# VincentStimper/normalizing-flows

Measured on NVIDIA H100. Metric: samples/sec forward_kld, 32-layer RQ-NSF d=64 batch=65536, higher is better.
Workload: dtype f32

## Files before the change

### normalizing-flows_b200/csrc/nfb_fused_rqs.cu

```cuda
#include <type_traits>

#include "nfb_kernels.h"
#include "nfb_spline.cuh"

namespace nfb {

constexpr int kRows = kFusedTileRows;
constexpr int kCons = 256;
constexpr int kFusedThreads = kCons + 128;
constexpr int kProducerRegs = 24, kConsumerRegs = 240;
constexpr uint32_t kTileA = 8192;
constexpr uint32_t kSlotBytes = 32768;
constexpr uint32_t kSlots = 3;
constexpr uint32_t kOffW = 8 * kTileA;
constexpr uint32_t kOffX = kOffW + kSlots * kSlotBytes;
constexpr int kStgLd = 52;
constexpr uint32_t kStgBytes = kRows * kStgLd * 4;
constexpr uint32_t kOffStg = kOffX + kRows * 64 * 4;
constexpr uint32_t kOffMisc = kOffStg + 2 * kStgBytes;
constexpr uint32_t kOffBars = kOffMisc + 4 * kRows * 4;
constexpr uint32_t kNumBars = 10;
constexpr uint32_t kOffUnitQ = kOffBars + kNumBars * 8;
constexpr uint32_t kFusedSmem = kOffUnitQ + 32;
static_assert(kFusedSmem <= 232448, "shared memory budget");
static_assert(2 * kFusedFeaturesPerChunk * 24 * 64 * 4 <= (int)kSlotBytes, "final-layer record must fit a ring slot");

constexpr int kBarWFull = 0 , kBarWEmpty = 3 , kBarUnit = 6 ;

__device__ __forceinline__ uint32_t xs_index(int r, int c) { return r * 64 + (c ^ (r & 31)); }

__device__ __forceinline__ uint32_t a_chunk_off(int r, int c8) {
    return (r >> 3) * 1024 + (r & 7) * 128 + ((c8 ^ (r & 7)) << 4);
}

__device__ __forceinline__ void st_shared_v4(uint32_t addr, uint32_t a, uint32_t b, uint32_t c,
                                             uint32_t d) {
    asm volatile("st.shared.v4.b32 [%0], {%1,%2,%3,%4};" ::"r"(addr), "r"(a), "r"(b), "r"(c), "r"(d)
                 : "memory");
}
__device__ __forceinline__ void st_shared_b32(uint32_t addr, uint32_t v) {
    asm volatile("st.shared.b32 [%0], %1;" ::"r"(addr), "r"(v) : "memory");
}
__device__ __forceinline__ void cons_bar_sync() {
    asm volatile("bar.sync 1, %0;" ::"n"(kCons) : "memory");
}
constexpr int kBarStgFull = 2, kBarStgFree = 3;
template <int ID> __device__ __forceinline__ void stg_bar_arrive() {
    __threadfence_block();
    asm volatile("bar.arrive %0, %1;" ::"n"(ID), "n"(kCons) : "memory");
}
template <int ID> __device__ __forceinline__ void stg_bar_wait() {
    asm volatile("bar.sync %0, %1;" ::"n"(ID), "n"(kCons) : "memory");
}
__device__ __forceinline__ void mbar_arrive_if(uint32_t bar, bool pred) {
    asm volatile("{\n\t.reg .pred p;\n\tsetp.ne.b32 p, %1, 0;\n\t@p mbarrier.arrive.shared::cta.b64 _, [%0];\n\t}"
                 ::"r"(bar), "r"((uint32_t)pred) : "memory");
}

__device__ __forceinline__ void split_store8(const float* v, uint32_t t0, uint32_t t1, uint32_t off) {
    uint32_t h[4], l[4];
#pragma unroll
    for (int i = 0; i < 4; ++i) {
        const float a = v[2 * i], b = v[2 * i + 1];
        h[i] = pack_f16x2(a, b);
        const float2 hf = unpack_f16x2(h[i]);
        l[i] = pack_f16x2(a - hf.x, b - hf.y);
    }
    st_shared_v4(t0 + off, h[0], h[1], h[2], h[3]);
    st_shared_v4(t1 + off, l[0], l[1], l[2], l[3]);
}
template <typename T> __device__ __forceinline__ T uniform(T v) {
    return (T)__shfl_sync(0xffffffffu, (int)v, 0);
}
__device__ __forceinline__ float pow2i(int e) { return __uint_as_float((uint32_t)(127 + e) << 23); }

struct MmaOps { uint32_t a_hi, a_lo, w_hi, w_lo; bool first; uint32_t on, slabs; };
template <int SLABS, bool QUAD, int NREG, bool FIRST = false>
__device__ __forceinline__ void mma_record(float (&acc)[NREG], const MmaOps& x) {
    static_assert(NREG == 32 || NREG == 48, "N = 64 or 96");
    static_assert(!FIRST || NREG == 48, "an opening record of its own: the final layer's N = 96 products");
    const uint64_t ah = wgmma_desc(x.a_hi), al = wgmma_desc(x.a_lo), bh = wgmma_desc(x.w_hi), bl = wgmma_desc(x.w_lo);
    auto pass = [&](uint64_t a, uint64_t b, bool opens) {
#pragma unroll
        for (int s = 0; s < SLABS; ++s) {
            const uint32_t sd = opens && s == 0 && x.first ? 0u : 1u;
            if constexpr (NREG == 32) wgmma_f16_n64(acc, a + 2 * s, b + 2 * s, sd);
            else if (FIRST && opens && s == 0) wgmma_f16_n96_zero(acc, a, b);
            else wgmma_f16_n96(acc, a + 2 * s, b + 2 * s, FIRST ? 1u : sd);
        }
    };
    pass(ah, bh, true);
    pass(al, bh, false);
    pass(ah, bl, false);
    if constexpr (QUAD) pass(al, bl, false);
}

enum { kClkClaim,
       kClkLoad,
       kClkLu,
       kClkHidRing,
       kClkHidMma,
       kClkHidEpi,
       kClkFinRing,
       kClkFinMma,
       kClkFinTail,
       kClkFinStage,
       kClkFinSpline,
       kClkStore,
       kClkProdEmpty,
       kClkProdOther,
       kClkUnits,
       kClkCount };
template <int P> using ClkPhase = std::integral_constant<int, P>;
#ifdef NFB_PHASE_CLOCKS
__device__ unsigned long long g_phase_clocks[3][kClkCount];
struct PhaseClock {
    uint32_t last, sum[kClkCount];
    __device__ PhaseClock() {
        last = (uint32_t)clock64();
#pragma unroll
        for (int i = 0; i < kClkCount; ++i) sum[i] = 0;
    }
    template <int P> __device__ __forceinline__ void stamp() {
        const uint32_t t = (uint32_t)clock64();
        sum[P] += t - last;
        last = t;
    }
    __device__ void flush(int role) const {
#pragma unroll
        for (int i = 0; i < kClkCount; ++i) atomicAdd(&g_phase_clocks[role][i], (unsigned long long)sum[i]);
    }
};
#define NFB_CLK_BEGIN() PhaseClock clk
#define NFB_CLK(P) clk.template stamp<P>()
#define NFB_CLK_UNIT() (++clk.sum[kClkUnits])
#define NFB_CLK_END(role, pred) do { if (pred) clk.flush(role); } while (0)
#else
#define NFB_CLK_BEGIN() ((void)0)
#define NFB_CLK(P) ((void)0)
#define NFB_CLK_UNIT() ((void)0)
#define NFB_CLK_END(role, pred) ((void)0)
#endif

template <bool SAMPLE>
__global__ void __launch_bounds__(kFusedThreads, 1) fused_rqs_kernel(const FusedParams p) {
    extern __shared__ __align__(1024) uint8_t smem[];
    const uint32_t sbase = smem_u32(smem);
    const int warp = uniform((int)(threadIdx.x >> 5)), lane = threadIdx.x & 31;
    float* xs = reinterpret_cast<float*>(smem + kOffX);
    float* ldsum = reinterpret_cast<float*>(smem + kOffMisc);
    int* rowexp = reinterpret_cast<int*>(smem + kOffMisc + 3 * kRows * 4);
    float* rowmax = reinterpret_cast<float*>(smem + kOffStg);
    const uint32_t bars = sbase + kOffBars;
    auto bar = [bars](int i) { return bars + 8u * i; };

    if ((sbase & 1023u) != 0) {
        if (threadIdx.x == 0 && p.err) atomicExch(p.err, 900);
        return;
    }
    if (threadIdx.x == 0) {
        for (int i = 0; i < (int)kSlots; ++i) {
            mbar_init(bar(kBarWFull + i), 1);
            mbar_init(bar(kBarWEmpty + i), 2);
        }
        for (int i = 0; i < 4; ++i) mbar_init(bar(kBarUnit + i), 1);
        fence_mbar_init();
    }
    __syncthreads();

    volatile int* unit_q = reinterpret_cast<volatile int*>(smem + kOffUnitQ);
    if (warp >= kCons / 32) {
        setmaxnreg_dec<kProducerRegs>();
        if (warp != kCons / 32) return;
        const long long n_tiles = (p.rows + kRows - 1) / kRows;
        const long long n_units = n_tiles * p.n_layers;
        auto decode = [&](long long u, int& cursor, int& layer, long long& tile) {
            if (!p.wave_order) {
                layer = (int)(u / n_tiles);
                tile = u - (long long)layer * n_tiles;
                return;
            }
            while (cursor + 1 < p.wave_elems && u >= (long long)__ldg(p.wave_order + 2 * (cursor + 1) + 1)) ++cursor;
            const uint32_t w = __ldg(p.wave_order + 2 * cursor);
            layer = (int)(w & 0xffu);
            tile = (long long)(w >> 8) * p.wave_tpg + (u - (long long)__ldg(p.wave_order + 2 * cursor + 1));
        };
        uint32_t slot = 0, par = 0;
        int wcur = 0;
        NFB_CLK_BEGIN();
        for (uint32_t ui = 0;; ++ui) {
            long long u;
            if (p.ticket) {
                int t = 0;
                if (lane == 0) t = atomicAdd(p.ticket, 1);
                u = (long long)__shfl_sync(0xffffffffu, t, 0);
            } else {
                u = (long long)blockIdx.x + (long long)ui * gridDim.x;
            }
            const bool more = u < n_units;
            int ulayer = -1;
            long long utile = 0;
            if (more) decode(u, wcur, ulayer, utile);
            if (lane == 0) {
                unit_q[2 * (ui & 3u)] = ulayer;
                unit_q[2 * (ui & 3u) + 1] = (int)utile;
                mbar_arrive(bar(kBarUnit + (ui & 3u)));
            }
            __syncwarp();
            if (!more) break;
            NFB_CLK_UNIT();
            const FusedLayer& L = p.layers[ulayer];
            const FusedStep* steps = L.steps;
            const int n_steps = L.n_steps;
            const int lu_steps = L.has_lu ? 1 : 0;
            const int reps = (SAMPLE && L.ar_passes > 0) ? L.ar_passes : 1;
            const int total = n_steps ? lu_steps + reps * (n_steps - lu_steps) : 0;
            const uint32_t lu_bytes = L.has_lu ? 2u * 8192u : 0u;
            int s = 0;
            uint32_t off = 0;
            uint32_t bytes = total ? (uint32_t)__ldg(&steps[0].bytes16) << 4 : 0u;
            for (int i = 0; i < total; ++i) {
                int sn = s + 1;
                uint32_t offn = off + bytes;
                if (sn == n_steps) { sn = lu_steps; offn = lu_bytes; }
                const uint32_t nbytes = i + 1 < total ? (uint32_t)__ldg(&steps[sn].bytes16) << 4 : 0u;
                NFB_CLK(kClkProdOther);
                mbar_wait(bar(kBarWEmpty + slot), par ^ 1, p.err, 100 + slot);
                NFB_CLK(kClkProdEmpty);
                if (elect_one_sync()) {
                    mbar_expect_tx(bar(kBarWFull + slot), bytes);
                    bulk_g2s(sbase + kOffW + slot * kSlotBytes, L.wstream + off, bytes, bar(kBarWFull + slot));
                }
                __syncwarp();
                s = sn;
                off = offn;
                bytes = nbytes;
                if (++slot == kSlots) { slot = 0; par ^= 1; }
            }
        }
        NFB_CLK(kClkProdOther);
        NFB_CLK_END(2, lane == 0);
        return;
    }

    setmaxnreg_inc<kConsumerRegs>();
    const int et = threadIdx.x;
    const int wg = uniform(et >> 7);
    const int wl = warp & 3;
    const int ra = 16 * wl + (lane >> 2);
    const int rb = ra + 8;
    const int cq = 2 * (lane & 3);
    const uint32_t aA = sbase;
    float* stg0 = reinterpret_cast<float*>(smem + kOffStg);
    uint32_t slot = 0, wpar = 0;
    NFB_CLK_BEGIN();

    for (uint32_t ui = 0;; ++ui) {
        mbar_wait(bar(kBarUnit + (ui & 3u)), (ui >> 2) & 1u, p.err, 600 + (int)(ui & 3u));
        const int layer = uniform(unit_q[2 * (ui & 3u)]);
        const long long tile = uniform(unit_q[2 * (ui & 3u) + 1]);
        if (layer < 0) break;
        NFB_CLK_UNIT();
        const FusedLayer& L = p.layers[layer];
        const int D = L.D;
        auto own = [&](int q) { return uniform((int)L.own[wg][q]); };
        const int n_steps = uniform(L.n_steps), lu_steps = uniform(L.has_lu ? 1 : 0);
        const int n_hidden = uniform(L.n_hidden), n_pairs = uniform(L.n_chunks >> 1);
        int sidx = 0;
        auto hand_back = [&](auto arrivals, int s, bool pred) {
#pragma unroll
            for (int i = 0; i < decltype(arrivals)::value; ++i) mbar_arrive_if(bar(kBarWEmpty + s), pred && (et & 127) == 0);
        };
        auto walk_records = [&](auto issue, auto arrivals, auto clk_ring, auto clk_mma, int& prev, auto open,
                                auto retire) {
            auto record = [&](auto first) {
                union { uint2 raw; FusedStep s; } st;
                st.raw = __ldg(reinterpret_cast<const uint2*>(L.steps) + sidx);
                st.raw.x = uniform(st.raw.x);
                st.raw.y = uniform(st.raw.y);
                sidx = sidx + 1 == n_steps ? lu_steps : sidx + 1;
                NFB_CLK(decltype(clk_mma)::value);
                mbar_wait(bar(kBarWFull + slot), wpar, p.err, 220 + slot);
                NFB_CLK(decltype(clk_ring)::value);
                wgmma_fence();
                const bool last = issue(st.s, first);
                if constexpr (decltype(first)::value) NFB_CLK(decltype(clk_mma)::value);
                wgmma_wait<1>();
                hand_back(arrivals, prev < 0 ? 0 : prev, prev >= 0);
                if constexpr (decltype(first)::value) NFB_CLK(kClkFinTail);
                prev = (int)slot;
                if (++slot == kSlots) { slot = 0; wpar ^= 1; }
                return last;
            };
            bool last = false;
            if constexpr (decltype(open)::value) {
                last = record(std::true_type());
                retire();
            }
            while (!last) last = record(std::false_type());
        };
        auto run_records = [&](auto issue, auto arrivals, auto clk_ring, auto clk_mma) {
            int prev = -1;
            walk_records(issue, arrivals, clk_ring, clk_mma, prev, std::false_type(), [] {});
            wgmma_wait<0>();
            hand_back(arrivals, prev, true);
            NFB_CLK(decltype(clk_mma)::value);
        };
        auto half_ops = [&](const FusedStep& s, int h, bool live) {
            const uint32_t kc = h ? s.kc1 : s.kc, fl = h ? s.flags1 : s.flags;
            const uint32_t w = sbase + kOffW + slot * kSlotBytes + ((fl & kStepHalf) ? 0u : (uint32_t)h * s.n8 * 1024u);
            return MmaOps{aA + kc * kTileA, aA + (4 + kc) * kTileA, w, w + ((uint32_t)s.bytes16 << 3), (fl & kStepFirst) != 0,
                          (uint32_t)(live && !(fl & kStepSkip)), 4u - ((fl >> kStepSlabShift) & 3u)};
        };
        auto run_slice = [&](auto& acc, bool live, auto quad, auto clk_ring, auto clk_mma) {
            run_records([&](const FusedStep& s, auto) {
                const MmaOps x = half_ops(s, wg, live);
                if (x.on) mma_record<4, decltype(quad)::value>(acc, x);
                wgmma_commit();
                return ((wg ? s.flags1 : s.flags) & kStepLast) != 0;
            }, std::integral_constant<int, 1>(), clk_ring, clk_mma);
            wgmma_hold(acc);
        };
        using NoQuad = std::integral_constant<bool, false>;

        float* zdst = p.zout + (long long)layer * p.z_stride;
        const float* zsrc = layer == 0 ? p.zin : p.zout + (long long)(layer - 1) * p.z_stride;
        const long long row0 = tile * kRows;
        const int r = et & (kRows - 1);
        const int rq = et >> 6;
        const long long grow = row0 + r;
        const bool row_live = grow < p.rows;

        if (layer > 0) {
            if (lane == 0) {
                const int* flag = p.progress + tile;
                int seen;
                const long long t0 = clock64();
                do {
                    asm volatile("ld.acquire.gpu.global.s32 %0, [%1];" : "=r"(seen) : "l"(flag) : "memory");
                    if (seen < layer && clock64() - t0 > 4000000000LL) fail_timeout(p.err, 500);
                } while (seen < layer);
            }
            __syncwarp();
            {
                int seen;
                asm volatile("ld.acquire.gpu.global.s32 %0, [%1];" : "=r"(seen) : "l"(p.progress + tile) : "memory");
                if (seen < layer) fail_timeout(p.err, 501);
            }
        }
        if (layer == 0 && p.in_ready) {
            const int need = (int)min(row0 + kRows, p.rows);
            if (lane == 0) {
                int seen;
                const long long t0 = clock64();
                do {
                    asm volatile("ld.acquire.sys.global.s32 %0, [%1];" : "=r"(seen) : "l"(p.in_ready) : "memory");
                    if (seen < need && clock64() - t0 > 20000000000LL) fail_timeout(p.err, 510);
                } while (seen < need);
            }
            __syncwarp();
            {
                int seen;
                asm volatile("ld.acquire.sys.global.s32 %0, [%1];" : "=r"(seen) : "l"(p.in_ready) : "memory");
                if (seen < need) fail_timeout(p.err, 511);
            }
        }
        NFB_CLK(kClkClaim);
        float lq_old = 0.f;
        if (rq == 2 && row_live && (layer > 0 || p.accumulate)) lq_old = __ldcg(p.logq + grow);
        if (D == 64) {
            float4 v[kRows * 16 / kCons];
#pragma unroll
            for (int k = 0; k < kRows * 16 / kCons; ++k) {
                const int i4 = et + k * kCons, rr = i4 >> 4;
                const long long gr = row0 + rr;
                v[k] = gr < p.rows ? __ldcg(reinterpret_cast<const float4*>(zsrc + gr * 64) + (i4 & 15))
                                   : make_float4(0.f, 0.f, 0.f, 0.f);
            }
#pragma unroll
            for (int k = 0; k < kRows * 16 / kCons; ++k) {
                const int i4 = et + k * kCons, rr = i4 >> 4, c0 = (i4 & 15) * 4;
                xs[xs_index(rr, c0)] = v[k].x;
                xs[xs_index(rr, c0 + 1)] = v[k].y;
                xs[xs_index(rr, c0 + 2)] = v[k].z;
                xs[xs_index(rr, c0 + 3)] = v[k].w;
                float m = fmaxf(fmaxf(fabsf(v[k].x), fabsf(v[k].y)), fmaxf(fabsf(v[k].z), fabsf(v[k].w)));
                m = fmaxf(m, __shfl_xor_sync(0xffffffffu, m, 1));
                m = fmaxf(m, __shfl_xor_sync(0xffffffffu, m, 2));
                m = fmaxf(m, __shfl_xor_sync(0xffffffffu, m, 4));
                m = fmaxf(m, __shfl_xor_sync(0xffffffffu, m, 8));
                if ((et & 15) == 0) rowmax[rr] = m;
            }
        } else {
            for (int i = et; i < kRows * D; i += kCons) {
                const int rr = i / D, cc = i - rr * D;
                const long long gr = row0 + rr;
                xs[xs_index(rr, cc)] = gr < p.rows ? __ldcg(zsrc + gr * D + cc) : 0.f;
            }
        }
        cons_bar_sync();
        auto set_row_exp = [&](float zmax) {
            int e = (int)((__float_as_uint(zmax) >> 23) & 0xffu) - 126;
            rowexp[r] = max(0, min(126, e));
        };
        if (rq == 0) {
            float zmax = 0.f;
            if (D == 64) zmax = rowmax[r];
            else
                for (int c = 0; c < D; ++c) zmax = fmaxf(zmax, fabsf(xs[xs_index(r, c)]));
            set_row_exp(zmax);
        }
        cons_bar_sync();
        auto ru = [&](float s, int row) { return s * pow2i(-rowexp[row]); };
        auto ruinv = [&](float s, int row) { return s * pow2i(rowexp[row]); };
        auto get_x = [&](int c) -> float { return xs[xs_index(r, c)]; };
        auto put_y = [&](int c, float y) { xs[xs_index(r, c)] = y; };
        const int ar = et >> 2, aq = et & 3;
        auto store_a = [&](auto value, float sc_base) {
            const float sc = ru(sc_base, ar);
            float v[16];
#pragma unroll
            for (int j = 0; j < 16; ++j) v[j] = value(aq * 16 + j) * sc;
#pragma unroll
            for (int g = 0; g < 2; ++g) split_store8(v + 8 * g, aA, aA + 4 * kTileA, a_chunk_off(ar, 2 * aq + g));
            fence_proxy_async_smem();
            cons_bar_sync();
        };
        auto build_a_net = [&]() {
            store_a([&](int k) {
                const int c = L.in_idx[k];
                return c >= 0 ? xs[xs_index(ar, c)] : 0.f;
            }, L.a_sc[1]);
        };
        float ladsum = 0.f, lad_even = 0.f;
        const bool folded = uniform(!SAMPLE && L.has_lu && L.fold_lu);
        if (lu_steps) {
            store_a([&](int k) { return k < D ? xs[xs_index(ar, k)] : 0.f; }, L.a_sc[0]);
            float acc[32];
            NFB_CLK(kClkLoad);
            run_slice(acc, wg == 0, std::integral_constant<bool, true>(), ClkPhase<kClkLu>(), ClkPhase<kClkLu>());
            if (wg == 0) {
                const float ia = ruinv(L.a_inv[0], ra), ib = ruinv(L.a_inv[0], rb);
#pragma unroll
                for (int i = 0; i < 32; ++i) {
                    const int c = 8 * (i >> 2) + cq + (i & 1);
                    const int rr = (i & 2) ? rb : ra;
                    if (c < D) xs[xs_index(rr, c)] = fmaf(acc[i], (i & 2) ? ib : ia, __ldg(L.bias_lu + c));
                }
            }
            cons_bar_sync();
            NFB_CLK(kClkLu);
        }
        auto store_tile = [&]() {
            if (D == 64) {
#pragma unroll
                for (int k = 0; k < kRows * 16 / kCons; ++k) {
                    const int i4 = et + k * kCons, rr = i4 >> 4, c0 = (i4 & 15) * 4;
                    const long long gr = row0 + rr;
                    const float4 v = make_float4(xs[xs_index(rr, c0)], xs[xs_index(rr, c0 + 1)],
                                                 xs[xs_index(rr, c0 + 2)], xs[xs_index(rr, c0 + 3)]);
                    if (gr < p.rows) __stcg(reinterpret_cast<float4*>(zdst + gr * 64) + (i4 & 15), v);
                }
            } else {
                for (int i = et; i < kRows * D; i += kCons) {
                    const int rr = i / D, cc = i - rr * D;
                    const long long gr = row0 + rr;
                    if (gr < p.rows) __stcg(zdst + gr * D + cc, xs[xs_index(rr, cc)]);
                }
            }
        };
        const bool arsamp = uniform(SAMPLE && L.ar_passes > 0);
        const int reps = uniform(arsamp ? L.ar_passes : 1);
        if (arsamp) {
            store_tile();
            if (rq == 0) {
                float zmax = L.tail;
                for (int c = 0; c < D; ++c) zmax = fmaxf(zmax, fabsf(xs[xs_index(r, c)]));
                set_row_exp(zmax);
            }
            cons_bar_sync();
            for (int i = et; i < kRows * 64; i += kCons) xs[i] = 0.f;
            cons_bar_sync();
        }
        for (int rep = 0; rep < reps; ++rep) {
            if (rep > 0) {
                ladsum = 0.f;
                cons_bar_sync();
            }
            auto uncond = [&]() {
                for (int i = rq; i < L.n_id; i += kCons / kRows) {
                    const int c = L.id_idx[i];
                    const float* tb = L.uncond + i * 23;
                    auto acc = [tb](int k) { return __ldg(tb + k); };
                    float y, l;
                    rqs_eval<8, SAMPLE>(get_x(c), acc, L.tail, 1.0f, y, l);
                    put_y(c, y);
                    ladsum += l;
                }
            };
            if (SAMPLE && L.n_id > 0) {
                uncond();
                cons_bar_sync();
            }
            if (!folded) build_a_net();
            if (!SAMPLE && L.n_id > 0) uncond();
            NFB_CLK(kClkLoad);

            if (wg == 0) ldsum[rq * kRows + r] = ladsum;
            float hres[2][32] = {};
            for (int ph = 0; ph < n_hidden; ++ph) {
                const bool t_phase = (ph & 1) != 0;
                const bool relu = ph + 1 < n_hidden;
                float tacc[2][32] = {};
#pragma unroll
                for (int q = 0; q < 2; ++q) {
                    const int j = own(q);
                    if (q == 0 || j >= 0) {
                        if (t_phase) run_slice(tacc[q], j >= 0, NoQuad(), ClkPhase<kClkHidRing>(), ClkPhase<kClkHidMma>());
                        else run_slice(hres[q], j >= 0, NoQuad(), ClkPhase<kClkHidRing>(), ClkPhase<kClkHidMma>());
                    }
                }
                cons_bar_sync();
                const float inv_a = ruinv(L.a_inv[1 + ph], ra), inv_b = ruinv(L.a_inv[1 + ph], rb);
                const float sc_a = ru(L.a_sc[2 + ph], ra), sc_b = ru(L.a_sc[2 + ph], rb);
                auto epilogue = [&](const float (&acc)[32], int j) {
                    const float* bias = L.bias_h + ph * 256 + 64 * j;
#pragma unroll
                    for (int g = 0; g < 8; ++g) {
                        const float2 b2 = __ldg(reinterpret_cast<const float2*>(bias + 8 * g + cq));
#pragma unroll
                        for (int hb = 0; hb < 2; ++hb) {
                            const int rr = hb ? rb : ra;
                            float v0 = fmaf(acc[4 * g + 2 * hb], hb ? inv_b : inv_a, b2.x);
                            float v1 = fmaf(acc[4 * g + 2 * hb + 1], hb ? inv_b : inv_a, b2.y);
                            if (relu) { v0 = fmaxf(v0, 0.f); v1 = fmaxf(v1, 0.f); }
                            v0 *= hb ? sc_b : sc_a;
                            v1 *= hb ? sc_b : sc_a;
                            const uint32_t hi = pack_f16x2(v0, v1);
                            const float2 hf = unpack_f16x2(hi);
                            const uint32_t off = (rr >> 3) * 1024 + (rr & 7) * 128 + ((g ^ (rr & 7)) << 4) + cq * 2;
                            st_shared_b32(aA + j * kTileA + off, hi);
                            st_shared_b32(aA + (4 + j) * kTileA + off, pack_f16x2(v0 - hf.x, v1 - hf.y));
                        }
                    }
                };
#pragma unroll
                for (int q = 0; q < 2; ++q) {
                    const int j = own(q);
                    if (j >= 0) {
                        if (t_phase) epilogue(tacc[q], j);
                        else epilogue(hres[q], j);
                    }
                }
                fence_proxy_async_smem();
                cons_bar_sync();
                NFB_CLK(kClkHidEpi);
            }

            if (wg == 0) {
                static_assert(kFusedFeaturesPerChunk == 2, "a final-layer record is one N = 96 product");
                auto products = [&](float (&acc)[48]) {
                    return [&](const FusedStep& s, auto first) {
                        constexpr bool F = decltype(first)::value;
                        const MmaOps x = half_ops(s, 0, true), x1 = half_ops(s, 1, true);
                        const uint32_t n = max(x.on ? x.slabs : 0u, x1.on ? x1.slabs : 0u);
                        switch (n) {
                            case 1: mma_record<1, false, 48, F>(acc, x); wgmma_commit(); break;
                            case 2: mma_record<2, false, 48, F>(acc, x); wgmma_commit(); break;
                            case 3: mma_record<3, false, 48, F>(acc, x); wgmma_commit(); break;
                            default: mma_record<4, false, 48, F>(acc, x); wgmma_commit(); break;
                        }
                        return (s.flags & kStepLast) != 0;
                    };
                };
                const float fin_a = ruinv(L.a_inv[1 + n_hidden], ra), fin_b = ruinv(L.a_inv[1 + n_hidden], rb);
                float2 fbias[2][6];
                auto load_bias = [&](int ci) {
                    if (ci >= n_pairs) return;
#pragma unroll
                    for (int h = 0; h < 2; ++h)
#pragma unroll
                        for (int g = 0; g < 6; ++g)
                            fbias[h][g] = __ldg(reinterpret_cast<const float2*>(L.bias_f + (2 * ci + h) * L.F * 24 + 8 * g + cq));
                };
                auto stage = [&](float (&acc)[48], int ci) {
                    wgmma_hold(acc);
                    if (ci > 0) stg_bar_wait<kBarStgFree>();
#pragma unroll
                    for (int i = 0; i < 24; i += 2) {
                        const int g = i >> 2;
                        const float u = (i & 2) ? fin_b : fin_a;
                        float* dst = stg0 + ((i & 2) ? rb : ra) * kStgLd + 8 * g + cq;
                        *reinterpret_cast<float2*>(dst) =
                            make_float2(fmaf(acc[i], u, fbias[0][g].x), fmaf(acc[i + 1], u, fbias[0][g].y));
                        *reinterpret_cast<float2*>(dst + kRows * kStgLd) =
                            make_float2(fmaf(acc[24 + i], u, fbias[1][g].x), fmaf(acc[25 + i], u, fbias[1][g].y));
                    }
                    stg_bar_arrive<kBarStgFull>();
                    load_bias(ci + 1);
                    NFB_CLK(kClkFinStage);
                };
                using Two = std::integral_constant<int, 2>;
                int prev = -1;
                auto pair = [&](float (&acc)[48], float (&done)[48], int ci) {
                    walk_records(products(acc), Two(), ClkPhase<kClkFinRing>(), ClkPhase<kClkFinMma>(), prev,
                                 std::true_type(), [&] { stage(done, ci - 1); });
                };
                auto finish = [&](float (&acc)[48], int ci) {
                    wgmma_wait<0>();
                    hand_back(Two(), prev, true);
                    NFB_CLK(kClkFinTail);
                    stage(acc, ci);
                };
                float accA[48], accB[48];
                if (n_pairs > 0) {
                    load_bias(0);
                    walk_records(products(accA), Two(), ClkPhase<kClkFinRing>(), ClkPhase<kClkFinMma>(), prev,
                                 std::true_type(), [] {});
                    for (int ci = 1;; ci += 2) {
                        if (ci == n_pairs) { finish(accA, ci - 1); break; }
                        pair(accB, accA, ci);
                        if (ci + 1 == n_pairs) { finish(accB, ci); break; }
                        pair(accA, accB, ci + 1);
                    }
                }
            } else {
                if (n_pairs > 0) {
                    const uint32_t adv = slot + (uint32_t)(n_steps - sidx);
                    slot = adv % kSlots;
                    wpar ^= (adv / kSlots) & 1u;
                    sidx = lu_steps;
                }
                const int f = (et >> 6) & 1;
                lad_even = ldsum[f * kRows + r];
                const int F = L.F, T = L.T;
                for (int ci = 0; ci < n_pairs; ++ci) {
                    stg_bar_wait<kBarStgFull>();
                    float pv[2][24];
#pragma unroll
                    for (int h = 0; h < 2; ++h) {
                        const float4* sp = reinterpret_cast<const float4*>(stg0 + (h * kRows + r) * kStgLd + 24 * f);
#pragma unroll
                        for (int q = 0; q < 6; ++q) {
                            const float4 s4 = sp[q];
                            pv[h][4 * q] = s4.x;
                            pv[h][4 * q + 1] = s4.y;
                            pv[h][4 * q + 2] = s4.z;
                            pv[h][4 * q + 3] = s4.w;
                        }
                    }
                    if (ci + 1 < n_pairs) stg_bar_arrive<kBarStgFree>();
                    NFB_CLK(kClkFinStage);
                    const int t0 = 2 * ci * F + f;
                    auto splines = [&](auto lanes) {
                        constexpr int N = decltype(lanes)::value;
                        int col[N];
                        float xin[N], y[N], l[N];
#pragma unroll
                        for (int h = 0; h < N; ++h) {
                            col[h] = L.tr_idx[t0 + h * F];
                            xin[h] = get_x(col[h]);
                            if (arsamp) xin[h] = row_live ? __ldcg(zdst + grow * D + col[h]) : 0.f;
                        }
                        rqs_core_lanes<N, 8, SAMPLE>(xin, [&pv](int h, int i) { return pv[h][i]; },
                                                     [&pv](int h, int i) { return pv[h][8 + i]; },
                                                     [&pv](int h, int i) { return pv[h][16 + i]; }, L.tail, y, l);
#pragma unroll
                        for (int h = 0; h < N; ++h) put_y(col[h], y[h]);
                        lad_even += l[0];
                        if constexpr (N == 2) ladsum += l[1];
                    };
                    if (t0 + F < T) splines(std::integral_constant<int, 2>());
                    else if (t0 < T) splines(std::integral_constant<int, 1>());
                    NFB_CLK(kClkFinSpline);
                }
            }
            cons_bar_sync();
        }
        NFB_CLK(kClkFinStage);
        if (rq == 3) {
            ldsum[r] = lad_even;
            ldsum[kRows + r] = ladsum;
        }
        cons_bar_sync();
        if (rq == 2 && row_live) {
            const float tot = lad_even + ldsum[r] + ladsum + ldsum[kRows + r] +
                              (L.lu_logdet ? __ldg(L.lu_logdet) : 0.f);
            __stcg(p.logq + grow, tot + lq_old);
        }
        store_tile();
        if (p.progress) __threadfence();
        cons_bar_sync();
        if (p.progress && et == 0) {
            __threadfence();
            asm volatile("st.release.gpu.global.s32 [%0], %1;" ::"l"(p.progress + tile), "r"(layer + 1) : "memory");
        }
        NFB_CLK(kClkStore);
    }
    NFB_CLK_END(wg, (et & 127) == 0);
}

int launch_fused_rqs(const FusedParams& p, int sm_count, int sample, cudaStream_t st) {
    static PerDevice per_dev;
    const int dev_sms = per_dev.ensure([] {
        cudaError_t e = cudaFuncSetAttribute(fused_rqs_kernel<false>, cudaFuncAttributeMaxDynamicSharedMemorySize,
                                             (int)kFusedSmem);
        if (e == cudaSuccess)
            e = cudaFuncSetAttribute(fused_rqs_kernel<true>, cudaFuncAttributeMaxDynamicSharedMemorySize, (int)kFusedSmem);
        return e;
    });
    if (dev_sms < 0) return NFB_ERR_CUDA;
    if (sm_count <= 0 || sm_count > dev_sms) sm_count = dev_sms;
    NFB_CHECK(p.n_layers >= 1 && (p.n_layers == 1 || p.progress), NFB_ERR_ARG, "fused rqs: bad layer list");
    const long long n_tiles = (p.rows + kRows - 1) / kRows;
    if (n_tiles == 0) return NFB_OK;
    const long long n_units = n_tiles * p.n_layers;
    const unsigned grid = (unsigned)(n_units < sm_count ? n_units : sm_count);
    if (sample) fused_rqs_kernel<true><<<grid, kFusedThreads, kFusedSmem, st>>>(p);
    else fused_rqs_kernel<false><<<grid, kFusedThreads, kFusedSmem, st>>>(p);
    NFB_LAUNCH_CHECK();
    return NFB_OK;
}

#ifdef NFB_PHASE_CLOCKS
extern "C" __attribute__((visibility("default"))) int nfb_phase_clocks_read(unsigned long long* out, int reset) {
    NFB_CUDA(cudaDeviceSynchronize());
    if (out) NFB_CUDA(cudaMemcpyFromSymbol(out, g_phase_clocks, sizeof(g_phase_clocks)));
    if (reset) {
        const unsigned long long zero[3][kClkCount] = {};
        NFB_CUDA(cudaMemcpyToSymbol(g_phase_clocks, zero, sizeof(zero)));
    }
    return NFB_OK;
}
extern "C" __attribute__((visibility("default"))) int nfb_phase_clocks_count() { return kClkCount; }
#endif

__global__ void build_effective_kernel(const float* __restrict__ W, const float* __restrict__ M,
                                       int src_cols, const int* __restrict__ src_row,
                                       const int* __restrict__ src_col,
                                       const float* __restrict__ row_scale, float* __restrict__ E,
                                       int n_pad, int k_pad, float gain) {
    const int idx = blockIdx.x * blockDim.x + threadIdx.x;
    if (idx >= n_pad * k_pad) return;
    const int i = idx / k_pad, j = idx - i * k_pad;
    const int sr = src_row[i], sc = src_col[j];
    float v = 0.f;
    if (sr >= 0 && sc >= 0) {
        const long long o = (long long)sr * src_cols + sc;
        v = W[o];
        if (M) v *= M[o];
        if (row_scale) v *= row_scale[i];
        v *= gain;
    }
    E[idx] = v;
}
__global__ void swizzle_split_kernel(const float* __restrict__ E, int n_pad, int k_pad,
                                     int rows_per_rec, int nsplit, float scale, uint8_t* __restrict__ out) {
    const int kcs = k_pad / 64;
    const long long total = (long long)n_pad * k_pad;
    const long long idx = (long long)blockIdx.x * blockDim.x + threadIdx.x;
    if (idx >= total) return;
    const int i = (int)(idx / k_pad), j = (int)(idx - (long long)i * k_pad);
    const int rb = i / rows_per_rec, rr = i - rb * rows_per_rec;
    const int kc = j >> 6, kk = j & 63;
    const float v = E[idx] * scale;
    const size_t rec_bytes = (size_t)rows_per_rec * 128;
    const size_t in_rec = (size_t)(rr >> 3) * 1024 + (rr & 7) * 128 + (((kk >> 3) ^ (rr & 7)) << 4) +
                          (kk & 7) * 2;
    float rem = v;
    for (int s = 0; s < nsplit; ++s) {
        const __half h = __float2half_rn(rem);
        rem -= __half2float(h);
        const size_t rec = ((size_t)rb * kcs + kc) * nsplit + s;
        *reinterpret_cast<__half*>(out + rec * rec_bytes + in_rec) = h;
    }
}

__global__ void pack_records_kernel(const float* __restrict__ E, int k_pad, const PackRec* __restrict__ recs, float scale,
                                    uint8_t* __restrict__ base) {
    const PackRec r = recs[blockIdx.y];
    const int idx = blockIdx.x * blockDim.x + threadIdx.x;
    if (idx >= r.nrows * 64) return;
    const int rr = idx >> 6, kk = idx & 63;
    const float v = E[(size_t)(r.row0 + rr) * k_pad + r.kc * 64 + kk] * scale;
    const size_t off = (size_t)(rr >> 3) * 1024 + (rr & 7) * 128 + (((kk >> 3) ^ (rr & 7)) << 4) + (kk & 7) * 2;
    const __half h = __float2half_rn(v);
    *reinterpret_cast<__half*>(base + r.off_hi + off) = h;
    *reinterpret_cast<__half*>(base + r.off_lo + off) = __float2half_rn(v - __half2float(h));
}
int launch_pack_records(const float* E, int k_pad, const PackRec* recs_dev, int n_recs, int max_rows, float scale,
                        uint8_t* base, cudaStream_t st) {
    if (n_recs == 0) return NFB_OK;
    NFB_CHECK(max_rows > 0 && max_rows % 8 == 0, NFB_ERR_ARG, "pack_records: bad row count %d", max_rows);
    const dim3 grid((unsigned)((max_rows * 64 + 255) / 256), (unsigned)n_recs);
    pack_records_kernel<<<grid, 256, 0, st>>>(E, k_pad, recs_dev, scale, base);
    NFB_LAUNCH_CHECK();
    return NFB_OK;
}
__global__ void fold_lu_kernel(const float* __restrict__ E0, const float* __restrict__ Elu, const float* __restrict__ blu,
                               const int* __restrict__ in_idx, int d, float gain, float* __restrict__ G,
                               float* __restrict__ delta) {
    const int i = blockIdx.x, c = threadIdx.x;
    double acc = 0.0;
    for (int k = 0; k < 64; ++k) {
        const int src = in_idx[k];
        if (src < 0 || src >= d) continue;
        const double w = (double)E0[(size_t)i * 64 + k];
        acc += w * (c < 64 ? (double)Elu[(size_t)src * 64 + c] : (double)blu[src]);
    }
    if (c < 64) G[(size_t)i * 64 + c] = (float)(acc * (double)gain);
    else delta[i] = (float)acc;
}
int launch_fold_lu(const float* E0, const float* Elu, const float* blu, const int* in_idx, int H, int d, float gain,
                   float* G, float* delta, cudaStream_t st) {
    fold_lu_kernel<<<H, 65, 0, st>>>(E0, Elu, blu, in_idx, d, gain, G, delta);
    NFB_LAUNCH_CHECK();
    return NFB_OK;
}

__global__ void matrix_norms_kernel(const float* __restrict__ E, int n, int k, float* __restrict__ out) {
    const int row = blockIdx.x;
    float sp = 0.f, sn = 0.f, mx = 0.f;
    for (int j = threadIdx.x; j < k; j += blockDim.x) {
        const float v = E[(size_t)row * k + j];
        sp += fmaxf(v, 0.f);
        sn += fmaxf(-v, 0.f);
        mx = fmaxf(mx, fabsf(v));
    }
    __shared__ float s[3][4];
    sp = warp_sum(sp);
    sn = warp_sum(sn);
#pragma unroll
    for (int o = 16; o > 0; o >>= 1) mx = fmaxf(mx, __shfl_xor_sync(0xffffffffu, mx, o));
    const int w = threadIdx.x >> 5;
    if ((threadIdx.x & 31) == 0) { s[0][w] = sp; s[1][w] = sn; s[2][w] = mx; }
    __syncthreads();
    if (threadIdx.x == 0) {
        float p = 0.f, q = 0.f, m = 0.f;
        for (int i = 0; i < (int)(blockDim.x >> 5); ++i) { p += s[0][i]; q += s[1][i]; m = fmaxf(m, s[2][i]); }
        atomicMax(reinterpret_cast<int*>(out), __float_as_int(p + q));
        atomicMax(reinterpret_cast<int*>(out + 1), __float_as_int(fmaxf(p, q)));
        atomicMax(reinterpret_cast<int*>(out + 2), __float_as_int(m));
    }
    (void)n;
}
int launch_matrix_norms(const float* E, int n, int k, float* out3, cudaStream_t st) {
    NFB_CUDA(cudaMemsetAsync(out3, 0, 3 * sizeof(float), st));
    matrix_norms_kernel<<<n, 128, 0, st>>>(E, n, k, out3);
    NFB_LAUNCH_CHECK();
    return NFB_OK;
}

int launch_build_effective(const float* W, const float* M, int src_cols, const int* src_row,
                           const int* src_col, const float* row_scale, float* E, int n_pad,
                           int k_pad, float gain, cudaStream_t st) {
    const int n = n_pad * k_pad;
    build_effective_kernel<<<(n + 255) / 256, 256, 0, st>>>(W, M, src_cols, src_row, src_col,
                                                            row_scale, E, n_pad, k_pad, gain);
    NFB_LAUNCH_CHECK();
    return NFB_OK;
}
int launch_swizzle_split(const float* E, int n_pad, int k_pad, int rows_per_rec, int nsplit, float scale,
                         uint8_t* out, cudaStream_t st) {
    NFB_CHECK(n_pad % rows_per_rec == 0 && k_pad % 64 == 0 && rows_per_rec % 8 == 0, NFB_ERR_ARG,
              "swizzle_split: bad shape %d x %d / %d", n_pad, k_pad, rows_per_rec);
    const long long n = (long long)n_pad * k_pad;
    swizzle_split_kernel<<<(unsigned)((n + 255) / 256), 256, 0, st>>>(E, n_pad, k_pad, rows_per_rec,
                                                                      nsplit, scale, out);
    NFB_LAUNCH_CHECK();
    return NFB_OK;
}

}
```

Before: 5.366 million.

## Stage hidden/LU biases in shared memory and drain wgmma once per phase

Hidden-layer and LU biases are now loaded into shared memory while the input tile is being loaded, and the epilogues read them from there instead of global memory. The two accumulator slices of a hidden phase are now walked back to back with a single final wgmma drain, rather than each slice waiting for all its MMAs. The aim is to remove an extra full wgmma wait between the slices and the per-epilogue global bias loads. In exchange it uses more shared memory and holds more accumulators live, which adds register pressure.

```diff
diff --git a/normalizing-flows_b200/csrc/nfb_fused_rqs.cu b/normalizing-flows_b200/csrc/nfb_fused_rqs.cu
--- a/normalizing-flows_b200/csrc/nfb_fused_rqs.cu
+++ b/normalizing-flows_b200/csrc/nfb_fused_rqs.cu
@@ -21,7 +21,11 @@
 constexpr uint32_t kOffBars = kOffMisc + 4 * kRows * 4;
 constexpr uint32_t kNumBars = 10;
 constexpr uint32_t kOffUnitQ = kOffBars + kNumBars * 8;
-constexpr uint32_t kFusedSmem = kOffUnitQ + 32;
+constexpr uint32_t kOffBiasH = kOffUnitQ + 32;
+constexpr int kBiasHVec = (int)sizeof(FusedLayer::bias_h) / 16;
+constexpr uint32_t kOffBiasLu = kOffBiasH + 16 * kBiasHVec;
+constexpr uint32_t kFusedSmem = kOffBiasLu + 64 * 4;
+static_assert(kOffBiasH % 16 == 0, "float4 copies of the hidden biases");
 static_assert(kFusedSmem <= 232448, "shared memory budget");
 static_assert(2 * kFusedFeaturesPerChunk * 24 * 64 * 4 <= (int)kSlotBytes, "final-layer record must fit a ring slot");
 
@@ -299,11 +303,10 @@
             }
             while (!last) last = record(std::false_type());
         };
-        auto run_records = [&](auto issue, auto arrivals, auto clk_ring, auto clk_mma) {
-            int prev = -1;
-            walk_records(issue, arrivals, clk_ring, clk_mma, prev, std::false_type(), [] {});
+        using One = std::integral_constant<int, 1>;
+        auto drain = [&](int prev, auto clk_mma) {
             wgmma_wait<0>();
-            hand_back(arrivals, prev, true);
+            hand_back(One(), prev, true);
             NFB_CLK(decltype(clk_mma)::value);
         };
         auto half_ops = [&](const FusedStep& s, int h, bool live) {
@@ -312,14 +315,17 @@
             return MmaOps{aA + kc * kTileA, aA + (4 + kc) * kTileA, w, w + ((uint32_t)s.bytes16 << 3), (fl & kStepFirst) != 0,
                           (uint32_t)(live && !(fl & kStepSkip)), 4u - ((fl >> kStepSlabShift) & 3u)};
         };
-        auto run_slice = [&](auto& acc, bool live, auto quad, auto clk_ring, auto clk_mma) {
-            run_records([&](const FusedStep& s, auto) {
+        auto walk_slice = [&](auto& acc, bool live, auto quad, auto clk_ring, auto clk_mma, int& prev) {
+            walk_records([&](const FusedStep& s, auto) {
                 const MmaOps x = half_ops(s, wg, live);
-                if (x.on) mma_record<4, decltype(quad)::value>(acc, x);
-                wgmma_commit();
+                if (x.on) {
+                    mma_record<4, decltype(quad)::value>(acc, x);
+                    wgmma_commit();
+                } else {
+                    wgmma_commit();
+                }
                 return ((wg ? s.flags1 : s.flags) & kStepLast) != 0;
-            }, std::integral_constant<int, 1>(), clk_ring, clk_mma);
-            wgmma_hold(acc);
+            }, One(), clk_ring, clk_mma, prev, std::false_type(), [] {});
         };
         using NoQuad = std::integral_constant<bool, false>;
 
@@ -368,6 +374,16 @@
         NFB_CLK(kClkClaim);
         float lq_old = 0.f;
         if (rq == 2 && row_live && (layer > 0 || p.accumulate)) lq_old = __ldcg(p.logq + grow);
+        constexpr int kBiasVecPerThread = (kBiasHVec + kCons - 1) / kCons;
+        float4 bias_v[kBiasVecPerThread];
+        float* bias_lu_s = reinterpret_cast<float*>(smem + kOffBiasLu);
+        float bias_lu_v = 0.f;
+#pragma unroll
+        for (int k = 0; k < kBiasVecPerThread; ++k) {
+            const int i = et + k * kCons;
+            if (i < n_hidden * 64) bias_v[k] = __ldg(reinterpret_cast<const float4*>(L.bias_h) + i);
+        }
+        if (lu_steps && et < 64) bias_lu_v = __ldg(L.bias_lu + et);
         if (D == 64) {
             float4 v[kRows * 16 / kCons];
 #pragma unroll
@@ -398,6 +414,12 @@
                 xs[xs_index(rr, cc)] = gr < p.rows ? __ldcg(zsrc + gr * D + cc) : 0.f;
             }
         }
+#pragma unroll
+        for (int k = 0; k < kBiasVecPerThread; ++k) {
+            const int i = et + k * kCons;
+            if (i < n_hidden * 64) reinterpret_cast<float4*>(smem + kOffBiasH)[i] = bias_v[k];
+        }
+        if (lu_steps && et < 64) bias_lu_s[et] = bias_lu_v;
         cons_bar_sync();
         auto set_row_exp = [&](float zmax) {
             int e = (int)((__float_as_uint(zmax) >> 23) & 0xffu) - 126;
@@ -438,14 +460,17 @@
             store_a([&](int k) { return k < D ? xs[xs_index(ar, k)] : 0.f; }, L.a_sc[0]);
             float acc[32];
             NFB_CLK(kClkLoad);
-            run_slice(acc, wg == 0, std::integral_constant<bool, true>(), ClkPhase<kClkLu>(), ClkPhase<kClkLu>());
+            int prev = -1;
+            walk_slice(acc, wg == 0, std::true_type(), ClkPhase<kClkLu>(), ClkPhase<kClkLu>(), prev);
+            const float ia = ruinv(L.a_inv[0], ra), ib = ruinv(L.a_inv[0], rb);
+            drain(prev, ClkPhase<kClkLu>());
+            wgmma_hold(acc);
             if (wg == 0) {
-                const float ia = ruinv(L.a_inv[0], ra), ib = ruinv(L.a_inv[0], rb);
 #pragma unroll
                 for (int i = 0; i < 32; ++i) {
                     const int c = 8 * (i >> 2) + cq + (i & 1);
                     const int rr = (i & 2) ? rb : ra;
-                    if (c < D) xs[xs_index(rr, c)] = fmaf(acc[i], (i & 2) ? ib : ia, __ldg(L.bias_lu + c));
+                    if (c < D) xs[xs_index(rr, c)] = fmaf(acc[i], (i & 2) ? ib : ia, bias_lu_s[c]);
                 }
             }
             cons_bar_sync();
@@ -512,22 +537,31 @@
                 const bool t_phase = (ph & 1) != 0;
                 const bool relu = ph + 1 < n_hidden;
                 float tacc[2][32] = {};
-#pragma unroll
-                for (int q = 0; q < 2; ++q) {
-                    const int j = own(q);
-                    if (q == 0 || j >= 0) {
-                        if (t_phase) run_slice(tacc[q], j >= 0, NoQuad(), ClkPhase<kClkHidRing>(), ClkPhase<kClkHidMma>());
-                        else run_slice(hres[q], j >= 0, NoQuad(), ClkPhase<kClkHidRing>(), ClkPhase<kClkHidMma>());
-                    }
-                }
-                cons_bar_sync();
+                wgmma_hold(tacc[0]);
+                wgmma_hold(tacc[1]);
+                const int own_j[2] = {own(0), own(1)};
                 const float inv_a = ruinv(L.a_inv[1 + ph], ra), inv_b = ruinv(L.a_inv[1 + ph], rb);
                 const float sc_a = ru(L.a_sc[2 + ph], ra), sc_b = ru(L.a_sc[2 + ph], rb);
+                int prev = -1;
+#pragma unroll
+                for (int q = 0; q < 2; ++q) {
+                    const int j = own_j[q];
+                    if (q == 0 || j >= 0) {
+                        if (t_phase) walk_slice(tacc[q], j >= 0, NoQuad(), ClkPhase<kClkHidRing>(), ClkPhase<kClkHidMma>(), prev);
+                        else walk_slice(hres[q], j >= 0, NoQuad(), ClkPhase<kClkHidRing>(), ClkPhase<kClkHidMma>(), prev);
+                    }
+                }
+                drain(prev, ClkPhase<kClkHidMma>());
+                wgmma_hold(tacc[0]);
+                wgmma_hold(tacc[1]);
+                wgmma_hold(hres[0]);
+                wgmma_hold(hres[1]);
+                cons_bar_sync();
                 auto epilogue = [&](const float (&acc)[32], int j) {
-                    const float* bias = L.bias_h + ph * 256 + 64 * j;
+                    const float* bias = reinterpret_cast<const float*>(smem + kOffBiasH) + ph * 256 + 64 * j;
 #pragma unroll
                     for (int g = 0; g < 8; ++g) {
-                        const float2 b2 = __ldg(reinterpret_cast<const float2*>(bias + 8 * g + cq));
+                        const float2 b2 = *reinterpret_cast<const float2*>(bias + 8 * g + cq);
 #pragma unroll
                         for (int hb = 0; hb < 2; ++hb) {
                             const int rr = hb ? rb : ra;
@@ -546,7 +580,7 @@
                 };
 #pragma unroll
                 for (int q = 0; q < 2; ++q) {
-                    const int j = own(q);
+                    const int j = own_j[q];
                     if (j >= 0) {
                         if (t_phase) epilogue(tacc[q], j);
                         else epilogue(hres[q], j);
```

After: 5.503 million, median of 6. 2.6% higher.
